# modelscope/FunASR

Measured on AMD Instinct MI355X. Metric: audio-seconds/sec (RTF^-1) Paraformer-large 30s@bs64, higher is better.
Workload: dtype f32 (GEMM / self-attention operands split into 2 fp16 planes, 3 fp16 MFMA products, f32 accumulate; all else f32)

## Files before the change

funasr_amd/_lib.py:

```python
from __future__ import annotations

import ctypes as C
import os
import subprocess
import threading

_HERE = os.path.dirname(os.path.abspath(__file__))
LIB_PATH = os.environ.get("PF_LIB_PATH") or os.path.join(_HERE, "libparaformer_hip.so")
CSRC_DIR = os.path.join(_HERE, "csrc")

ABI_VERSION = 5

_lock = threading.Lock()
_lib = None


class HipRuntimeError(RuntimeError):
    """A pf_* entry point returned a non-zero status."""


class pf_frontend_config(C.Structure):
    _fields_ = [
        ("sample_rate", C.c_int32), ("frame_length", C.c_int32), ("frame_shift", C.c_int32),
        ("n_mels", C.c_int32), ("lfr_m", C.c_int32), ("lfr_n", C.c_int32),
# ... 112 lines not shown
    "pf_predictor_destroy": (None, [_vp]),
    "pf_predictor_set_tensor": (C.c_int, [_vp, C.c_char_p, _vp, _i64]),
    "pf_predictor_missing": (C.c_int, [_vp]),
    "pf_predictor_alphas": (C.c_int, [_vp, _vp, _pi32, _i32, _i32, _vp, _vp, _pi32, _vp]),
    "pf_predictor_embeds": (C.c_int, [_vp, _vp, _i32, _i32, _i32, _vp, _vp]),
    "pf_predictor_alphas_begin": (C.c_int, [_vp, _i32, _vp, _pi32, _i32, _i32, _vp, _vp, _vp, _vp]),
    "pf_predictor_embeds_slot": (C.c_int, [_vp, _i32, _vp, _i32, _i32, _i32, _vp, _vp]),
    "pf_predictor_create_v3": (_vp, [C.POINTER(pf_predictor_config), C.POINTER(pf_predictor_v3_config)]),
    "pf_predictor_timestamp": (C.c_int, [_vp, _vp, _pi32, _pi32, _i32, _i32, _vp, _vp, _vp]),
    "pf_decoder_create": (_vp, [C.POINTER(pf_decoder_config)]),
    "pf_decoder_destroy": (None, [_vp]),
    "pf_decoder_set_decoders2": (C.c_int, [_vp, _i32]),
    "pf_decoder_set_tensor": (C.c_int, [_vp, C.c_char_p, _vp, _i64]),
    "pf_decoder_missing": (C.c_int, [_vp]),
    "pf_decoder_set_precision": (C.c_int, [_vp, _i32]),
    "pf_decoder_forward": (C.c_int, [_vp, _vp, _pi32, _vp, _pi32, _i32, _i32, _i32, _vp, _vp, _vp, _vp]),
    "pf_decoder_create_contextual": (_vp, [C.POINTER(pf_decoder_config)]),
    "pf_decoder_forward_contextual": (C.c_int, [_vp, _vp, _pi32, _vp, _pi32, _vp, _i32, _f32, _i32, _i32, _i32, _vp, _vp, _vp, _vp]),
    "pf_decoder_asf_scores": (C.c_int, [_vp, _vp, _pi32, _vp, _pi32, _i32, _i32, _i32, _i32, _vp, _vp]),
    "pf_vad_create": (_vp, [C.POINTER(pf_vad_config)]),
    "pf_vad_destroy": (None, [_vp]),
    "pf_vad_set_tensor": (C.c_int, [_vp, C.c_char_p, _vp, _i64]),
    "pf_vad_missing": (C.c_int, [_vp]),
    "pf_vad_forward": (C.c_int, [_vp, _vp, _i32, _i32, _vp, _pi32, _i32, _vp, _vp, _i32, _vp]),
    "pf_vad_frame_decibel": (C.c_int, [_vp, _i64, _i32, _i32, _i32, _vp, _vp]),
    "pf_vad_decision_create": (_vp, [C.POINTER(pf_vad_options)]),
    "pf_vad_decision_destroy": (None, [_vp]),
    "pf_vad_decision_set_thresholds": (None, [_vp, C.c_double, C.c_double]),
    "pf_vad_decision_state": (C.c_int, [_vp]),
    "pf_vad_decision_push": (C.c_int, [_vp, _vp, _vp, _i32, _i32, _i32, _vp, _i32]),
# ... 160 lines not shown
```

funasr_amd/csrc/attention_f16x2.hip:

```cpp
#include "common.h"

namespace pf {

namespace {

constexpr int DK = 128, KT = 32;
constexpr int KP_B = KT * DK * 2;
constexpr int VP_B = DK * KT * 2;
constexpr int STAGE_B = 2 * KP_B + 2 * VP_B;
constexpr int OLD = DK + 4;
constexpr int SLAB_B = 8 * 32 * OLD * 4;
constexpr int LDS_BYTES = SLAB_B > 3 * STAGE_B ? SLAB_B : 3 * STAGE_B;
constexpr float P_SCALE = 1024.f;
typedef _Float16 f16x8 __attribute__((ext_vector_type(8)));

constexpr float LAZY_TAU = 3.0f;
template <int PIPE, bool LAZY = false>
__global__ __launch_bounds__(512, 2) void attention_f16x2_kernel(Attn2Args p) {
    extern __shared__ __attribute__((aligned(16))) unsigned char smem[];
    constexpr int NSTAGE = PIPE ? 3 : 2;
    constexpr int QB = 256;
    constexpr int NV = 1;

    const int tid = threadIdx.x, lane = tid & 63;
    const int wave = __builtin_amdgcn_readfirstlane(tid >> 6);
    const int hh = lane >> 5, idx = lane & 31;
    int b, head, qblk;
    if (p.xcd_nqb > 0) {
        const int L = blockIdx.x, j = L >> 3;
        const int pair = (j / p.xcd_nqb) * 8 + (L & 7);
        if (pair >= p.B * p.H) return;
        qblk = j % p.xcd_nqb; head = pair % p.H; b = pair / p.H;
    } else {
        b = blockIdx.z; head = blockIdx.y; qblk = blockIdx.x;
    }
    const int Tq = p.qoffs ? p.qoffs[b + 1] - p.qoffs[b] : (p.Tq > 0 ? p.Tq : p.Tp);
    if (qblk * QB >= Tq) return;
// ... 44 lines not shown
            glds16(vsrc[v] + kt * KT, base + 2 * KP_B);
            glds16(vsrc[v] + p.vt_plane + kt * KT, base + 2 * KP_B + VP_B);
        }
    };

    const float sscale = p.sscale_dev ? p.sscale * *p.sscale_dev : p.sscale;
    const float sscale2 = LAZY ? sscale * 1.4426950408889634f : sscale;
#define PF_EXP(x_) (LAZY ? __builtin_amdgcn_exp2f(x_) : __expf(x_))
    constexpr float PSC = LAZY ? 1.f : P_SCALE;
    const int ntiles = (kend + KT - 1) / KT;

#define PF_QK(KT_, SA, SB)                                                                                            \
    {                                                                                                                 \
        const unsigned char* kp = smem + ((KT_) % NSTAGE) * STAGE_B + idx * 256;                                      \
        _Pragma("unroll") for (int r = 0; r < 16; ++r) { SA[r] = 0.f; SB[r] = 0.f; }                                  \
        _Pragma("unroll") for (int st = 0; st < 8; ++st) {                                                            \
            const int co = ((2 * st + hh) ^ (idx & 15)) * 16;                                                         \
            const f16x8 kh = __builtin_bit_cast(f16x8, *reinterpret_cast<const uint4*>(kp + co));                     \
            const f16x8 kl = __builtin_bit_cast(f16x8, *reinterpret_cast<const uint4*>(kp + KP_B + co));              \
            SA = __builtin_amdgcn_mfma_f32_32x32x16_f16(kl, qf[0][st], SA, 0, 0, 0);                                  \
            SB = __builtin_amdgcn_mfma_f32_32x32x16_f16(kh, qf[0][st], SB, 0, 0, 0);                                  \
            SA = __builtin_amdgcn_mfma_f32_32x32x16_f16(kh, qf[1][st], SA, 0, 0, 0);                                  \
        }                                                                                                             \
    }
#define PF_SOFTMAX(K0_, SA, SB)                                                                                       \
    {                                                                                                                 \
        float mx = -INFINITY;                                                                                         \
        if (LAZY && (K0_) >= kskip && (K0_) + KT <= kend) {         \
            _Pragma("unroll") for (int r = 0; r < 16; ++r) {                                                          \
                s[r] = (SA[r] + SB[r]) * sscale2;                                                                     \
                mx = fmaxf(mx, s[r]);                                                                                 \
            }                                                                                                         \
        } else {                                                                                                      \
            _Pragma("unroll") for (int r = 0; r < 16; ++r) {                                                          \
                const int key = (K0_) + (r & 3) + 8 * (r >> 2) + 4 * hh;                                              \
                s[r] = (unsigned)(key - kskip) < (unsigned)klen ? (SA[r] + SB[r]) * sscale2 : -INFINITY;              \
                mx = fmaxf(mx, s[r]);                                                                                 \
            }                                                                                                         \
        }                                                                                                             \
        mx = fmaxf(mx, __shfl_xor(mx, 32, 64));                                                                       \
        float m_new = fmaxf(m_run, mx);                                                                               \
// ... 5 lines not shown
        const float alpha = moved ? PF_EXP(m_run - m_new) : 1.f;                                                      \
        float psum = 0.f;                                                                                             \
        const float m_off = LAZY ? m_new - 10.f : m_new;          \
        _Pragma("unroll") for (int r = 0; r < 16; ++r) {                                                              \
            s[r] = PF_EXP(s[r] - m_off);                                                                              \
            psum += s[r];                                                                                             \
        }                                                                                                             \
        psum += __shfl_xor(psum, 32, 64);                                                                             \
        l_run = l_run * alpha + psum;                                                                                 \
        m_run = m_new;                                                                                                \
        if (!LAZY || __any(moved)) {                                                                                  \
            _Pragma("unroll") for (int d = 0; d < 4; ++d) _Pragma("unroll") for (int r = 0; r < 16; ++r) o[d][r] *= alpha; \
        }                                                                                                             \
    }
#define PF_PV(KT_)                                                                                                    \
    {                                                                                                                 \
        const unsigned char* vp = smem + ((KT_) % NSTAGE) * STAGE_B + 2 * KP_B + idx * 64;                            \
        _Pragma("unroll") for (int st = 0; st < 2; ++st) {                                                            \
            uint4 ph, pl;                                                                                             \
            split2_pk(s[8 * st + 0] * PSC, s[8 * st + 1] * PSC, ph.x, pl.x);                                  \
            split2_pk(s[8 * st + 2] * PSC, s[8 * st + 3] * PSC, ph.y, pl.y);                                  \
            split2_pk(s[8 * st + 4] * PSC, s[8 * st + 5] * PSC, ph.z, pl.z);                                  \
            split2_pk(s[8 * st + 6] * PSC, s[8 * st + 7] * PSC, ph.w, pl.w);                                  \
            const f16x8 Ph = __builtin_bit_cast(f16x8, ph), Pl = __builtin_bit_cast(f16x8, pl);                       \
            const int co = ((2 * st + hh) ^ ((idx >> 2) & 3)) * 16;                                                   \
            f16x8 vf[4][2];                                                                                           \
            _Pragma("unroll") for (int d = 0; d < 4; ++d) _Pragma("unroll") for (int pn = 0; pn < 2; ++pn)            \
                vf[d][pn] = __builtin_bit_cast(f16x8, *reinterpret_cast<const uint4*>(vp + pn * VP_B + d * 32 * 64 + co)); \
            _Pragma("unroll") for (int d = 0; d < 4; ++d) o[d] = __builtin_amdgcn_mfma_f32_32x32x16_f16(vf[d][1], Ph, o[d], 0, 0, 0); \
            _Pragma("unroll") for (int d = 0; d < 4; ++d) o[d] = __builtin_amdgcn_mfma_f32_32x32x16_f16(vf[d][0], Pl, o[d], 0, 0, 0); \
            _Pragma("unroll") for (int d = 0; d < 4; ++d) o[d] = __builtin_amdgcn_mfma_f32_32x32x16_f16(vf[d][0], Ph, o[d], 0, 0, 0); \
        }                                                                                                             \
    }

    float s[16];
    const bool active = qblk * QB + wave * 32 < Tq;
    if constexpr (PIPE == 0) {
        stage(0);
        for (int kt = 0; kt < ntiles; ++kt) {
            glds_wait_all();
            __syncthreads();
            if (kt + 1 < ntiles) stage(kt + 1);
            if (active) {
                floatx16 sa, sb;
                PF_QK(kt, sa, sb)
                PF_SOFTMAX(kt * KT, sa, sb)
                PF_PV(kt)
            }
        }
    } else {
        floatx16 ca, cb, na, nb;
        stage(0);
        if (ntiles > 1) stage(1);
        glds_wait_all();
        __syncthreads();
        PF_QK(0, ca, cb)
        for (int kt = 0; kt < ntiles; ++kt) {
            if (kt > 0) { glds_wait_all(); __syncthreads(); }
            if (kt + 2 < ntiles) stage(kt + 2);
            const int kn = kt + 1 < ntiles ? kt + 1 : kt;
            PF_QK(kn, na, nb)
            PF_SOFTMAX(kt * KT, ca, cb)
#pragma unroll
            for (int g = 0; g < 24; ++g) {
                __builtin_amdgcn_sched_group_barrier(0x008, 1, 0);
                __builtin_amdgcn_sched_group_barrier(0x002, 7, 0);
            }
            PF_PV(kt)
            ca = na; cb = nb;
        }
    }
#undef PF_QK
#undef PF_EXP
#undef PF_SOFTMAX
#undef PF_PV

    __syncthreads();
    float* slab = reinterpret_cast<float*>(smem) + wave * (32 * OLD);
    {
        const float inv = (LAZY ? p.oscale * P_SCALE : p.oscale) / l_run;
#pragma unroll
        for (int d = 0; d < 4; ++d)
#pragma unroll
            for (int g = 0; g < 4; ++g) {
                const float4 t = make_float4(o[d][4 * g + 0] * inv, o[d][4 * g + 1] * inv, o[d][4 * g + 2] * inv, o[d][4 * g + 3] * inv);
                *reinterpret_cast<float4*>(slab + idx * OLD + d * 32 + 8 * g + 4 * hh) = t;
            }
    }
    const int qw0 = qblk * QB + wave * 32;
#pragma unroll
    for (int it = 0; it < 8; ++it) {
        const int rr = it * 4 + (lane >> 4), c8 = (lane & 15) * 8;
// ... 2 lines not shown
        if (qw0 + rr < Tq) {
            uint4 h, l;
            split2_pk(a.x, a.y, h.x, l.x);
            split2_pk(a.z, a.w, h.y, l.y);
            split2_pk(c.x, c.y, h.z, l.z);
            split2_pk(c.z, c.w, h.w, l.w);
            unsigned short* op = p.O + (qrow0 + qw0 + rr) * p.ldo + head * DK + c8;
            *reinterpret_cast<uint4*>(op) = h;
            *reinterpret_cast<uint4*>(op + p.o_plane) = l;
        }
    }
}

}

int launch_attention_f16x2(const Attn2Args& a, hipStream_t stream) {
    PF_REQUIRE(a.B > 0 && a.H > 0 && (a.koffs || (a.Tp > 0 && a.Tp % 16 == 0)), "attention_f16x2: rows per sequence must be a positive multiple of 16");
    PF_REQUIRE(a.ldq % 8 == 0 && a.ldk % 8 == 0 && a.ldvt % 8 == 0 && a.ldo % 8 == 0 && a.q_plane % 8 == 0 &&
               a.k_plane % 8 == 0 && a.vt_plane % 8 == 0 && a.o_plane % 8 == 0, "attention_f16x2: strides % 8");
    PF_REQUIRE(((uintptr_t)a.Q & 15) == 0 && ((uintptr_t)a.K & 15) == 0 && ((uintptr_t)a.VT & 15) == 0 && ((uintptr_t)a.O & 15) == 0,
               "attention_f16x2: 16-B alignment");
    static PerDeviceOnce configured;
    if (!configured.done()) {
#if defined(PF_MEASUREMENT_KERNELS)
        PF_HIP_TRY(hipFuncSetAttribute(reinterpret_cast<const void*>(&attention_f16x2_kernel<0>),
                                       hipFuncAttributeMaxDynamicSharedMemorySize, LDS_BYTES));
        PF_HIP_TRY(hipFuncSetAttribute(reinterpret_cast<const void*>(&attention_f16x2_kernel<1>),
                                       hipFuncAttributeMaxDynamicSharedMemorySize, LDS_BYTES));
#endif
        PF_HIP_TRY(hipFuncSetAttribute(reinterpret_cast<const void*>(&attention_f16x2_kernel<0, true>),
                                       hipFuncAttributeMaxDynamicSharedMemorySize, LDS_BYTES));
        configured.mark();
    }
    const int rows = a.Tq > 0 ? a.Tq : a.Tp;
    Attn2Args k = a;
#if defined(PF_MEASUREMENT_KERNELS)
    PF_REQUIRE(a.variant == 0 || a.variant == 1 || a.variant == 3, "attention_f16x2: variant must be 0, 1 or 3");
#else
    PF_REQUIRE(a.variant == 3, "attention_f16x2: variant must be 3 (variants 0 / 1: the measurement library, make measure)");
#endif
    const int nqb = ceil_div(rows, 256);
    dim3 grid(nqb, a.H, a.B);
    k.xcd_nqb = (a.xcd_nqb >= 0 && nqb > 1) ? nqb : 0;
    if (k.xcd_nqb > 0) grid = dim3((unsigned)(ceil_div(a.B * a.H, 8) * 8 * nqb), 1, 1);
    if (a.variant == 3)
        hipLaunchKernelGGL((attention_f16x2_kernel<0, true>), grid, dim3(512), LDS_BYTES, stream, k);
#if defined(PF_MEASUREMENT_KERNELS)
    else if (a.variant == 1)
        hipLaunchKernelGGL(attention_f16x2_kernel<1>, grid, dim3(512), LDS_BYTES, stream, k);
    else
        hipLaunchKernelGGL(attention_f16x2_kernel<0>, grid, dim3(512), LDS_BYTES, stream, k);
#endif
    PF_HIP_TRY(hipGetLastError());
    return 0;
}

}
```

funasr_amd/csrc/common.h:

```cpp
#pragma once
#include <hip/hip_runtime.h>
#include <stdint.h>
#include <stdio.h>
#include <string>
#include <atomic>

typedef float floatx16 __attribute__((ext_vector_type(16)));
typedef float floatx4 __attribute__((ext_vector_type(4)));

namespace pf {

inline int current_device_slot() {
    int d = 0;
    if (hipGetDevice(&d) != hipSuccess || d < 0) d = 0;
    return d & 63;
}
struct PerDeviceOnce {
    std::atomic<bool> flag[64];
    PerDeviceOnce() { for (auto& f : flag) f.store(false, std::memory_order_relaxed); }
    bool done() const { return flag[current_device_slot()].load(std::memory_order_acquire); }
    void mark() { flag[current_device_slot()].store(true, std::memory_order_release); }
};
inline int device_cu_count() {
    static std::atomic<int> n[64];
// ... 344 lines not shown
struct Attn2Args {
    const unsigned short* Q; int ldq; size_t q_plane;
    const unsigned short* K; int ldk; size_t k_plane;
    const unsigned short* VT; int ldvt; size_t vt_plane;
    unsigned short* O; int ldo; size_t o_plane;
    const int* klens;
    int B, H, Tp;
    int Tq;
    float sscale;
    const float* sscale_dev;
    float oscale;
    int variant;
    const int* qoffs;
    int xcd_nqb;
    const int* koffs;
};
int launch_attention_f16x2(const Attn2Args& a, hipStream_t stream);

int launch_asf_scores(const float* Q, int ldq, const float* K, int ldk, float* P_scratch, float* out, int H, int dk, int N, int T,
                      int klen, float scale, hipStream_t stream);
bool attention_small_applicable(const AttnArgs& a, int dk);
int launch_attention_small(const AttnArgs& a, int dk, hipStream_t stream);
int launch_scatter_i32(const int* in, const int* map, int* out, int n, hipStream_t stream);
int launch_gather_rows(const float* table, int ld, int rows, const int* ids, float* out, int n, int D, hipStream_t stream);

int launch_vad_fsmn(const float* x, int ldx, const float* w, const float* cache_in, float* cache_out, float* y, int ldy,
                    int B, int T, int C, int L, int S, hipStream_t stream);
int launch_vad_softmax_sil(const float* x, int ldx, int M, int N, const int* ids, int n_ids, float* p_sil, float* probs,
                           int ldp, hipStream_t stream);
int launch_frame_decibel(const float* wav, int n_frames, int flen, int shift, float* out, hipStream_t stream);
// ... 3 lines not shown
```

funasr_amd/csrc/engine_decoder.hip:

```cpp
#include "engine_internal.h"

namespace pf {

std::string dec_layer_prefix(bool contextual, int n_blocks, int i) {
    return (contextual && i == n_blocks - 1) ? std::string("last_decoder.") : "decoders." + std::to_string(i) + ".";
}


int decoder_resolve(Decoder* d) {
    std::string first;
    const int miss = d->tt.missing(&first);
    if (miss) { set_error("decoder: " + std::to_string(miss) + " tensors not set, e.g. " + first); return -3; }
    d->layers.clear();
    for (int i = 0; i < d->cfg.n_blocks; ++i) {
        const std::string p = dec_layer_prefix(d->contextual, d->cfg.n_blocks, i);
        DecLayerW w;
        w.n1g = d->tt.get(p + "norm1.weight"); w.n1b = d->tt.get(p + "norm1.bias");
        w.w1 = d->tt.get(p + "feed_forward.w_1.weight"); w.b1 = d->tt.get(p + "feed_forward.w_1.bias");
        w.fng = d->tt.get(p + "feed_forward.norm.weight"); w.fnb = d->tt.get(p + "feed_forward.norm.bias");
        w.w2 = d->tt.get(p + "feed_forward.w_2.weight");
        w.n2g = d->tt.get(p + "norm2.weight"); w.n2b = d->tt.get(p + "norm2.bias");
        w.fsmn_w = d->tt.get(p + "self_attn.fsmn_block.weight");
        w.n3g = d->tt.get(p + "norm3.weight"); w.n3b = d->tt.get(p + "norm3.bias");
        w.q_w = d->tt.get(p + "src_attn.linear_q.weight"); w.q_b = d->tt.get(p + "src_attn.linear_q.bias");
// ... 627 lines not shown
    return 0;
}
int pf_decoder_set_tensor(pf_decoder* dh, const char* name, const float* data, int64_t numel) {
    Decoder* d = reinterpret_cast<Decoder*>(dh);
    PF_REQUIRE(d && name && data, "decoder_set_tensor: null");
    d->resolved = false;
    d->tt.drop_bf16();
    return d->tt.set(name, data, numel);
}
int pf_decoder_set_precision(pf_decoder* dh, int32_t mode) {
    Decoder* d = reinterpret_cast<Decoder*>(dh);
    PF_REQUIRE(d && mode >= 0 && mode <= 3, "decoder_set_precision: mode must be 0 (fp32 MFMA), 1 (bf16 operands), 2 (fp32 via bf16x3) or 3 (fp32 via f16x2)");
    d->precision = mode;
    return 0;
}
int pf_decoder_missing(const pf_decoder* dh) {
    const Decoder* d = reinterpret_cast<const Decoder*>(dh);
    return d ? d->tt.missing() : -1;
}

static int decoder_forward_impl(Decoder* d, const float* memory, const int32_t* mem_lens, const float* embeds,
                                const int32_t* tok_lens, int32_t B, int32_t T, int32_t N, float* logits, int32_t* ids,
                                float* hidden_out, hipStream_t s, int asf_layer, float* asf_scores, const DecCtxArgs* cx = nullptr);

int pf_decoder_forward(pf_decoder* dh, const float* memory, const int32_t* mem_lens, const float* embeds,
                       const int32_t* tok_lens, int32_t B, int32_t T, int32_t N, float* logits, int32_t* ids,
                       float* hidden_out, void* stream) {
    return decoder_forward_impl(reinterpret_cast<Decoder*>(dh), memory, mem_lens, embeds, tok_lens, B, T, N, logits, ids,
                                hidden_out, reinterpret_cast<hipStream_t>(stream), -1, nullptr);
}
// ... 152 lines not shown
                Gemm2Args g{};
                g.A = mem2; g.lda = D; g.a_plane = (size_t)Mkp * D; g.W = w.kv_2; g.ldw = D; g.w_plane = (size_t)2 * D * D;
                g.oscale = pow2f(-w.ew_kv); g.oscale_dev = dsc + 2; g.bias = w.kv_b; g.M = Mkp; g.N = 2 * D; g.K = D;
                g.qkv_D = D; g.kv_form = 1; g.Kp = k2; g.qk_plane = ((size_t)Mkp + 32) * D; g.VT = vt2; g.ldvt = Mkp + 64;
                g.vt_plane = (size_t)D * (Mkp + 64); g.k_mul = 1.f; g.v_mul = 1.f; g.kv_mul_dev = lsc;
                ProfScope ps(PROF_GEMM3, 2.0 * mem_rows * 2.0 * D * D, s);
                if ((rc = launch_gemm_f16x2(g, s))) return rc;
            }
            {
                Attn2Args aa{};
                aa.Q = d->q16.as<unsigned short>(); aa.ldq = D; aa.q_plane = (size_t)Mq * D;
                aa.K = k2; aa.ldk = D; aa.k_plane = ((size_t)Mkp + 32) * D; aa.VT = vt2; aa.ldvt = Mkp + 64;
                aa.vt_plane = (size_t)D * (Mkp + 64); aa.O = d->ctx16.as<unsigned short>(); aa.ldo = D; aa.o_plane = (size_t)Mq * D;
                aa.klens = d->mem_lens.as<int>(); aa.B = B; aa.H = c.n_heads; aa.Tp = Tp; aa.Tq = N; aa.qoffs = offs_dev;
                aa.sscale = pow2f(-w.e_q); aa.sscale_dev = lsc + 2; aa.oscale = pow2f(-10);
                aa.variant = 3;
                ProfScope ps(PROF_ATTN, 4.0 * tok_mem * D, s);
                if ((rc = launch_attention_f16x2(aa, s))) return rc;
            }
            if ((rc = gemm2_simple(d->ctx16.as<unsigned short>(), D, Mq, 0, w.o_2, w.ew_o, w.o_b, x, D, D, D, 0, x, D, s, lsc + 3)))
                return rc;
            continue;
        } else if (x3) {
            if ((rc = gemm3_simple(mem3, D, Mk, w3(lp + "src_attn.linear_k_v.weight", 2 * D, D), w.kv_b, d->kv.as<float>(),
                                   2 * D, 2 * D, D, 0, s))) return rc;
        } else if ((rc = gemm_simple(memory, D, w.kv_w, D, w.kv_b, d->kv.as<float>(), 2 * D, Mk, 2 * D, D, 0, nullptr, 0,
                                     nullptr, 0, s))) return rc;
        const bool ctx_block = cx && l == c.n_blocks - 1;
        if (ctx_block) {
            if (d->xself.ensure(sizeof(float) * (size_t)Mq * D) || d->xcat.ensure(sizeof(float) * (size_t)Mq * 2 * D)) return -2;
            PF_HIP_TRY(hipMemcpyAsync(d->xself.p, x, sizeof(float) * (size_t)Mq * D, hipMemcpyDeviceToDevice, s));
// ... 165 lines not shown
```

funasr_amd/csrc/engine_encoder.hip:

```cpp
#include "engine_internal.h"

namespace pf {

static void enc_layer_names(std::vector<std::pair<std::string, int>>& out, const pf_encoder_config& c) {
    out.push_back({"encoders0.0.", c.input_dim});
    for (int i = 0; i < c.n_blocks - 1; ++i) out.push_back({"encoders." + std::to_string(i) + ".", c.d_model});
    for (int i = 0; i < c.tp_blocks; ++i) out.push_back({"tp_encoders." + std::to_string(i) + ".", c.d_model});
}

int encoder_resolve(Encoder* e) {
    std::string first;
    const int miss = e->tt.missing(&first);
    if (miss) { set_error("encoder: " + std::to_string(miss) + " tensors not set, e.g. " + first); return -3; }
    std::vector<std::pair<std::string, int>> names;
    enc_layer_names(names, e->cfg);
    e->layers.clear();
    for (auto& nm : names) {
        const std::string& p = nm.first;
        EncLayerW w;
        w.prefix = p;
        w.in_dim = nm.second; w.in_pad = round_up(nm.second, 64);
        w.n1g = e->tt.get(p + "norm1.weight"); w.n1b = e->tt.get(p + "norm1.bias");
        w.qkv_w = e->tt.get(p + "self_attn.linear_q_k_v.weight"); w.qkv_b = e->tt.get(p + "self_attn.linear_q_k_v.bias");
        w.fsmn_w = e->tt.get(p + "self_attn.fsmn_block.weight");
// ... 443 lines not shown
int pf_encoder_set_option(pf_encoder* eh, const char* key, int32_t value) {
    Encoder* e = reinterpret_cast<Encoder*>(eh);
    PF_REQUIRE(e && key, "encoder_set_option: null");
    const std::string k = key;
    if (k == "fuse_row") { PF_REQUIRE(value == 0 || value == 1, "encoder_set_option: fuse_row is 0 or 1"); e->fuse_row = value; return 0; }
    if (k == "fsmn_fused") { PF_REQUIRE(value == 0 || value == 1, "encoder_set_option: fsmn_fused is 0 or 1"); e->fsmn_fused = value; return 0; }
    if (k == "w2_row") { PF_REQUIRE(value >= 0 && value <= 2, "encoder_set_option: w2_row is 0, 1 or 2"); e->w2_row = value; return 0; }
#if defined(PF_MEASUREMENT_KERNELS)
    if (k == "gemm_tile") { PF_REQUIRE(value == 0 || value == 1 || value == 2 || value == 5 || value == 6 || value == 7 || value == 8 || value == 9 || value == 10 || value == 12, "encoder_set_option: gemm_tile is 0, 1, 2, 5, 6, 7, 8, 9, 10 or 12"); e->gemm_tile = value; return 0; }
    if (k == "ffn_abl") { e->ffn_abl = value; return 0; }
    if (k == "ffn_fused") { PF_REQUIRE(value >= 0 && value <= 2, "encoder_set_option: ffn_fused is 0, 1 or 2"); e->ffn_fused = value; return 0; }
    if (k == "row_bm") { PF_REQUIRE(value == 0 || value == 96 || value == 128 || value == 129 || value == 130, "encoder_set_option: row_bm is 0, 96, 128, 129 or 130"); e->row_bm = value; return 0; }
    if (k == "row_sched") { PF_REQUIRE(value == 0 || value == 2, "encoder_set_option: row_sched is 0 or 2"); e->row_sched = value; return 0; }
    if (k == "w2_tile") { PF_REQUIRE(value == 0 || value == 2 || value == 7 || value == 8 || value == 10, "encoder_set_option: w2_tile is 0, 2, 7, 8 or 10"); e->w2_tile = value; return 0; }
    if (k == "row_nt") { PF_REQUIRE(value >= 0 && value <= 2, "encoder_set_option: row_nt is 0, 1 or 2"); e->row_nt = value; return 0; }
    if (k == "attn_variant") { PF_REQUIRE(value == 0 || value == 1 || value == 3, "encoder_set_option: attn_variant is 0, 1 or 3"); e->attn_variant = value; return 0; }
#else
    if (k == "gemm_tile") { PF_REQUIRE(value == 0 || value == 2 || value == 7 || value == 10, "encoder_set_option: gemm_tile is 0, 2, 7 or 10"); e->gemm_tile = value; return 0; }
    if (k == "ffn_abl" || k == "ffn_fused" || k == "row_bm" || k == "row_sched" || k == "w2_tile" || k == "row_nt" || k == "attn_variant") {
        set_error("encoder_set_option: " + k + " selects a measured-and-off shape: build and load the measurement library (make -C funasr_amd/csrc measure; PF_LIB_PATH)");
        return -1;
    }
#endif
    set_error("encoder_set_option: unknown key " + k);
    return -1;
}
static int poison(std::initializer_list<DevBuf*> bufs, int byte) {
    PF_HIP_TRY(hipDeviceSynchronize());
    for (DevBuf* b : bufs) if (b->p && b->cap) PF_HIP_TRY(hipMemset(b->p, byte, b->cap));
    PF_HIP_TRY(hipDeviceSynchronize());
    return 0;
}
int pf_encoder_debug_poison(pf_encoder* eh, int32_t byte) {
// ... 201 lines not shown
```

funasr_amd/csrc/engine_internal.h:

```cpp
#pragma once
#include <math.h>
#include <string.h>

#include <map>
#include <memory>
#include <mutex>
#include <string>
#include <vector>

#include "../../include/paraformer_hip.h"
#include "cif.h"
#include "lstm.h"
#include "common.h"
#include "frontend.h"
#include "stream.h"
#include "engine_tables.h"


namespace pf {

void set_error(const std::string& msg);
const char* get_error();

struct ProfRec { hipEvent_t a, b; int kind; double work; const char* tag; };
// ... 277 lines not shown
    bool vad_mask = false;
    std::vector<int32_t> h_vad;
    DevBuf vad_dev;
    int cur_mask_mode = 0;
    int fuse_row = 1;
    int fsmn_fused = 1;
    int ffn_fused = 0;
    int ffn_abl = 0;
    int row_bm = 0;
    int row_sched = 0;
    int w2_row = 2;
    int w2_tile = 7;
    DevBuf fs_grp;
    std::vector<int32_t> h_fs;
    const int* cur_fs = nullptr; int cur_fs_groups = 0;
    int attn_variant = 3;
    int row_nt = 1;
    double prof_rows = 0, prof_sq = 0;
    int gemm_tile = 0;
};


static inline int exp_for_bound(float bound) {
    if (!(bound > 0.f)) return 15;
    int e = (int)floorf(log2f(32768.f / bound));
    return e > 15 ? 15 : e;
}
static inline float pow2f(int e) { return ldexpf(1.f, e); }

static inline bool encoder_w2_row_form(const Encoder* e, int M) {
    if (e->w2_row != 2) return e->w2_row == 1;
// ... 50 lines not shown
};


struct Decoder {
    pf_decoder_config cfg;
    bool contextual = false;
    DevBuf xself, xcat, ctx_lens;
    TensorTable tt;
    std::vector<DecLayerW> layers;
    int n_blocks2 = 0;
    std::vector<DecLayerW> layers2;
    DecLayerW last;
    bool resolved = false;
    DevBuf x, t1, t2, ffn, ffn2, q, kv, ctx, mem_lens, tok_lens, pval, pidx, hid;
    int precision = 0;
    DevBuf t16, ffn16, ffn2_16, q16, kv16, ctx16, mem16, hid16;
    DevBuf dsc;
    DevBuf dscl, dlb;
    DevBuf k2, vt2;
    DevBuf splitk;
    bool lb_uploaded = false;
    int e_an = INT32_MIN;
    DevBuf asf_p;
    DevBuf offs_dev, map_dev, ids_packed;
    std::vector<int32_t> h_offs, h_map;
};


struct Ctc {
    int d_model, vocab;
// ... 117 lines not shown
```

funasr_amd/csrc/engine_kernels.hip:

```cpp
#include "engine_internal.h"

using namespace pf;

extern "C" {

int pf_k_gemm_skinny_ln(const float* A, int32_t lda, const float* W, int32_t ldw, const float* bias, const float* R2, int32_t ldr2,
                        float* Cout, int32_t ldc, int32_t M, int32_t N, int32_t K, int32_t relu, float* stats_out,
                        const float* stats_in, const float* ln_g, const float* ln_c, float ln_eps, const float* out_gamma, float* ws_part,
                        int32_t* ws_count, void* stream) {
    GemmArgs g{};
    g.ws_part = ws_part; g.ws_count = ws_count; g.ln_c1 = ln_c; g.ln_c2 = ln_c ? ln_c + N : nullptr; g.out_gamma = out_gamma;
    g.A = A; g.lda = lda; g.W = W; g.ldw = ldw; g.bias = bias; g.R2 = R2; g.ldr2 = ldr2; g.C = Cout; g.ldc = ldc;
    g.M = M; g.N = N; g.K = K; g.relu = relu; g.ln_stats_out = stats_out; g.ln_stats_in = stats_in; g.ln_g = ln_g; g.ln_eps = ln_eps;
    PF_REQUIRE(gemm_skinny_applicable(g), "gemm_skinny_ln: K % 16");
    return launch_gemm_skinny(g, reinterpret_cast<hipStream_t>(stream));
}
int pf_k_ln_consts(const float* W, int32_t ldw, int32_t N, int32_t K, const float* gamma, const float* beta, const float* bias, float* c,
                   void* stream) {
    return launch_ln_consts(W, ldw, N, K, gamma, beta, bias, c, c + N, reinterpret_cast<hipStream_t>(stream));
}
int pf_set_skinny_max_m(int32_t m) { g_skinny_max_m = m; return 0; }

int pf_k_gemm_f32(const float* A, int32_t lda, const float* W, int32_t ldw, const float* bias, const float* R1,
                  int32_t ldr1, const float* R2, int32_t ldr2, float* C, int32_t ldc, int32_t M, int32_t N, int32_t K,
// ... 121 lines not shown
    return 0;
}
int pf_k_attention_f16x2(const void* Q2, int64_t q_plane, const void* K2, int64_t k_plane, const void* VT2, int32_t ldvt,
                         int64_t vt_plane, void* O2, int64_t o_plane, const int32_t* klens_dev, int32_t B, int32_t H,
                         int32_t Tp, int32_t Tq, float sscale, float oscale, int32_t variant, int32_t iters, float* ms_out,
                         void* stream) {
    hipStream_t s = reinterpret_cast<hipStream_t>(stream);
    Attn2Args aa{};
    const int D = H * 128;
    aa.Q = reinterpret_cast<const unsigned short*>(Q2); aa.ldq = D; aa.q_plane = (size_t)q_plane;
    aa.K = reinterpret_cast<const unsigned short*>(K2); aa.ldk = D; aa.k_plane = (size_t)k_plane;
    aa.VT = reinterpret_cast<const unsigned short*>(VT2); aa.ldvt = ldvt; aa.vt_plane = (size_t)vt_plane;
    aa.O = reinterpret_cast<unsigned short*>(O2); aa.ldo = D; aa.o_plane = (size_t)o_plane;
    aa.klens = klens_dev; aa.B = B; aa.H = H; aa.Tp = Tp; aa.Tq = Tq; aa.sscale = sscale; aa.oscale = oscale;
    aa.variant = variant & 15; aa.xcd_nqb = (variant & 16) ? -1 : 0;
    int rc;
    if (iters <= 0 || !ms_out) return launch_attention_f16x2(aa, s);
    for (int i = 0; i < 3; ++i) if ((rc = launch_attention_f16x2(aa, s))) return rc;
    hipEvent_t a, b;
    PF_HIP_TRY(hipEventCreate(&a));
    PF_HIP_TRY(hipEventCreate(&b));
    PF_HIP_TRY(hipEventRecord(a, s));
    for (int i = 0; i < iters; ++i) if ((rc = launch_attention_f16x2(aa, s))) return rc;
    PF_HIP_TRY(hipEventRecord(b, s));
    PF_HIP_TRY(hipEventSynchronize(b));
    float ms = 0.f;
    PF_HIP_TRY(hipEventElapsedTime(&ms, a, b));
    (void)hipEventDestroy(a);
    (void)hipEventDestroy(b);
    *ms_out = ms / iters;
// ... 231 lines not shown
```

funasr_amd/paraformer_decoder.py:

```python
from __future__ import annotations

from typing import List

import torch
import torch.nn as nn

from . import _lib
from .hip_module import Holder, HipModule, ParamHolder, depthwise, device_lens, host_i32, layer_norm, linear, stream_ptr
from .register import tables


def _ffn(block, d_model, ffn):
    block.norm1 = layer_norm(d_model)
    block.feed_forward = Holder()
    block.feed_forward.w_1 = linear(ffn, d_model)
    block.feed_forward.norm = layer_norm(ffn)
    block.feed_forward.w_2 = linear(d_model, ffn, bias=False)


def _block2(d_model, ffn, kernel_size):
    b = Holder()
    _ffn(b, d_model, ffn)
    b.norm2 = layer_norm(d_model)
    b.self_attn = Holder()
# ... 49 lines not shown
        self.output_layer = linear(vocab_size, D) if use_output_layer else None

    def _default_precision(self) -> str:
        ok = self.d_model % 256 == 0 and self.d_model // self.attention_heads == 128 and self.linear_units % 256 == 0
        return "f16x2" if ok else "fp32"

    def _mode(self) -> str:
        return getattr(self, "_precision", None) or self._default_precision()

    def set_precision(self, mode=None):
        if mode is not None and mode not in ("fp32", "bf16", "bf16x3", "f16x2"):
            raise ValueError("precision must be 'fp32', 'bf16', 'bf16x3' or 'f16x2'")
        self._precision = mode
        return self

    def _make_config(self):
        return _lib.pf_decoder_config(self.vocab_size if self.output_layer is not None else 0, self.d_model, self.attention_heads, self.linear_units,
                                      self.att_layer_num, self.kernel_size, self.sanm_shfit, 1e-12)

    def _after_create(self, lib, handle):
        if self.decoders2 is not None:
            _lib.check(lib.pf_decoder_set_decoders2(handle, len(self.decoders2)), "pf_decoder_set_decoders2")

    def _apply_settings(self):
        lib, h = self._ensure_handle()
        _lib.check(lib.pf_decoder_set_precision(h, {"fp32": 0, "bf16": 1, "bf16x3": 2, "f16x2": 3}[self._mode()]),
                   "pf_decoder_set_precision")
        return lib, h

    def _run(self, hs_pad, hlens, ys_in_pad, ys_in_lens, want_logits: bool, want_ids: bool, want_hidden: bool = False):
        lib, h = self._apply_settings()
        dev = self._handle_device
        mem = hs_pad.to(device=dev, dtype=torch.float32).contiguous()
        emb = ys_in_pad.to(device=dev, dtype=torch.float32).contiguous()
        B, T, D = mem.shape
        N = emb.shape[1]
        mlen_c, _ = host_i32(hlens, B)
        tlen_c, tlens = host_i32(ys_in_lens, B)
        logits = torch.empty(B, N, self.vocab_size, device=dev, dtype=torch.float32) if want_logits else None
        ids = torch.empty(B, N, device=dev, dtype=torch.int32) if want_ids else None
        hid = torch.empty(B, N, D, device=dev, dtype=torch.float32) if want_hidden else None
        with torch.cuda.device(dev):
# ... 42 lines not shown
```

include/paraformer_hip.h:

```cpp
#ifndef PARAFORMER_HIP_H_
#define PARAFORMER_HIP_H_

#include <stdint.h>

#ifdef __cplusplus
extern "C" {
#endif

#define PF_ABI_VERSION 5

const char* pf_last_error(void);
int pf_abi_version(void);
int pf_device_count(void);

int pf_set_concurrency_guard(int32_t on);
int pf_concurrency_guard(void);

typedef struct pf_frontend pf_frontend;

typedef struct pf_frontend_config {
    int32_t sample_rate;
    int32_t frame_length;
    int32_t frame_shift;
    int32_t n_mels;
// ... 96 lines not shown
    int32_t d_model;
    int32_t n_heads;
    int32_t ffn_dim;
    int32_t n_blocks;
    int32_t kernel_size;
    int32_t sanm_shift;
    float ln_eps;
} pf_decoder_config;

pf_decoder* pf_decoder_create(const pf_decoder_config* cfg);
void pf_decoder_destroy(pf_decoder* d);
int pf_decoder_set_decoders2(pf_decoder* d, int32_t n_layers);
int pf_decoder_set_tensor(pf_decoder* d, const char* name, const float* data, int64_t numel);
int pf_decoder_missing(const pf_decoder* d);
int pf_decoder_set_precision(pf_decoder* d, int32_t mode);
int pf_decoder_forward(pf_decoder* d, const float* memory_dev, const int32_t* mem_lens_host,
                       const float* embeds_dev, const int32_t* tok_lens_host, int32_t B, int32_t T, int32_t N,
                       float* logits_dev, int32_t* ids_dev, float* hidden_dev, void* stream);
typedef struct pf_paraformer pf_paraformer;
pf_paraformer* pf_paraformer_create(pf_encoder* e, pf_predictor* p, pf_decoder* d);
void pf_paraformer_destroy(pf_paraformer* m);
int pf_paraformer_forward(pf_paraformer* m, const float* feats_dev, const int32_t* lens_host, int32_t B, int32_t T,
                          const float* pe_dev, int32_t* ids_dev, int32_t ids_ld, int32_t* token_num_host,
                          float* alphas_dev, float* peaks_dev, void* stream);
int pf_paraformer_begin(pf_paraformer* m, const float* feats_dev, const int32_t* lens_host, int32_t B, int32_t T,
                        const float* pe_dev, void* stream);
int pf_paraformer_finish(pf_paraformer* m, int32_t ticket, int32_t* ids_dev, int32_t ids_ld, int32_t* token_num_host,
                         float* alphas_dev, float* peaks_dev, void* stream);
const float* pf_paraformer_encoder_out(const pf_paraformer* m);
const float* pf_paraformer_embeds(const pf_paraformer* m);
// ... 251 lines not shown
```

Baseline: 39100.

## Add 4-wave attention variant with auto selection and batched K-fragment loads

Adds a 4-wave (128-query block) form of the f16x2 flash-attention kernel and a default variant 7 that picks it when the workgroup-round count across CUs favours smaller blocks, targeting tail and underfill waste at batch 64. The QK loop now loads four K fragment pairs before issuing their MFMAs, with sched_group_barrier hints, and the PV loop also gets these hints, to overlap LDS reads with matrix work. It also adds ablation and staggered-wave measurement variants, a decoder set_option entry point and host-side qlens for packed decoder rows. The heuristic uses a fixed 1.15 factor and the extra live fragments can raise register pressure.

```diff
diff --git a/funasr_amd/_lib.py b/funasr_amd/_lib.py
--- a/funasr_amd/_lib.py
+++ b/funasr_amd/_lib.py
@@ -150,6 +150,7 @@
     "pf_decoder_set_tensor": (C.c_int, [_vp, C.c_char_p, _vp, _i64]),
     "pf_decoder_missing": (C.c_int, [_vp]),
     "pf_decoder_set_precision": (C.c_int, [_vp, _i32]),
+    "pf_decoder_set_option": (C.c_int, [_vp, C.c_char_p, _i32]),
     "pf_decoder_forward": (C.c_int, [_vp, _vp, _pi32, _vp, _pi32, _i32, _i32, _i32, _vp, _vp, _vp, _vp]),
     "pf_decoder_create_contextual": (_vp, [C.POINTER(pf_decoder_config)]),
     "pf_decoder_forward_contextual": (C.c_int, [_vp, _vp, _pi32, _vp, _pi32, _vp, _i32, _f32, _i32, _i32, _i32, _vp, _vp, _vp, _vp]),
diff --git a/funasr_amd/csrc/attention_f16x2.hip b/funasr_amd/csrc/attention_f16x2.hip
--- a/funasr_amd/csrc/attention_f16x2.hip
+++ b/funasr_amd/csrc/attention_f16x2.hip
@@ -11,16 +11,19 @@
 constexpr int OLD = DK + 4;
 constexpr int SLAB_B = 8 * 32 * OLD * 4;
 constexpr int LDS_BYTES = SLAB_B > 3 * STAGE_B ? SLAB_B : 3 * STAGE_B;
+constexpr int SLAB4_B = 4 * 32 * OLD * 4;
+constexpr int LDS4_BYTES = SLAB4_B > 2 * STAGE_B ? SLAB4_B : 2 * STAGE_B;
 constexpr float P_SCALE = 1024.f;
 typedef _Float16 f16x8 __attribute__((ext_vector_type(8)));
 
 constexpr float LAZY_TAU = 3.0f;
-template <int PIPE, bool LAZY = false>
-__global__ __launch_bounds__(512, 2) void attention_f16x2_kernel(Attn2Args p) {
+template <int PIPE, bool LAZY = false, int NW = 8, int STAG = 0, int ABL = 0>
+__global__ __launch_bounds__(NW * 64, 2) void attention_f16x2_kernel(Attn2Args p) {
     extern __shared__ __attribute__((aligned(16))) unsigned char smem[];
-    constexpr int NSTAGE = PIPE ? 3 : 2;
-    constexpr int QB = 256;
-    constexpr int NV = 1;
+    static_assert((NW == 8 || NW == 4) && (STAG == 0 || (PIPE == 0 && NW == 8)), "attention_f16x2: form");
+    constexpr int NSTAGE = (PIPE || STAG == 1) ? 3 : 2;
+    constexpr int QB = NW * 32;
+    constexpr int NV = 8 / NW;
 
     const int tid = threadIdx.x, lane = tid & 63;
     const int wave = __builtin_amdgcn_readfirstlane(tid >> 6);
@@ -95,17 +98,37 @@
     {                                                                                                                 \
         const unsigned char* kp = smem + ((KT_) % NSTAGE) * STAGE_B + idx * 256;                                      \
         _Pragma("unroll") for (int r = 0; r < 16; ++r) { SA[r] = 0.f; SB[r] = 0.f; }                                  \
-        _Pragma("unroll") for (int st = 0; st < 8; ++st) {                                                            \
+        if constexpr (ABL & 4) { asm volatile("" : "+v"(SA), "+v"(SB)); }   \
+        else if constexpr (ABL & 64) { _Pragma("unroll") for (int st = 0; st < 8; ++st) {                             \
             const int co = ((2 * st + hh) ^ (idx & 15)) * 16;                                                         \
             const f16x8 kh = __builtin_bit_cast(f16x8, *reinterpret_cast<const uint4*>(kp + co));                     \
             const f16x8 kl = __builtin_bit_cast(f16x8, *reinterpret_cast<const uint4*>(kp + KP_B + co));              \
             SA = __builtin_amdgcn_mfma_f32_32x32x16_f16(kl, qf[0][st], SA, 0, 0, 0);                                  \
             SB = __builtin_amdgcn_mfma_f32_32x32x16_f16(kh, qf[0][st], SB, 0, 0, 0);                                  \
             SA = __builtin_amdgcn_mfma_f32_32x32x16_f16(kh, qf[1][st], SA, 0, 0, 0);                                  \
-        }                                                                                                             \
+        } }                                                                                                           \
+        else { _Pragma("unroll") for (int h4 = 0; h4 < 8; h4 += 4) {   \
+            f16x8 kh[4], kl[4];                                        \
+            _Pragma("unroll") for (int j = 0; j < 4; ++j) {                                                           \
+                const int co = ((2 * (h4 + j) + hh) ^ (idx & 15)) * 16;                                               \
+                kh[j] = __builtin_bit_cast(f16x8, *reinterpret_cast<const uint4*>(kp + co));                          \
+                kl[j] = __builtin_bit_cast(f16x8, *reinterpret_cast<const uint4*>(kp + KP_B + co));                   \
+            }                                                                                                         \
+            _Pragma("unroll") for (int j = 0; j < 4; ++j) {                                                           \
+                SA = __builtin_amdgcn_mfma_f32_32x32x16_f16(kl[j], qf[0][h4 + j], SA, 0, 0, 0);                       \
+                SB = __builtin_amdgcn_mfma_f32_32x32x16_f16(kh[j], qf[0][h4 + j], SB, 0, 0, 0);                       \
+                SA = __builtin_amdgcn_mfma_f32_32x32x16_f16(kh[j], qf[1][h4 + j], SA, 0, 0, 0);                       \
+            }                                                                                                         \
+             \
+            __builtin_amdgcn_sched_group_barrier(0x100, 8, 0);                                                        \
+            __builtin_amdgcn_sched_group_barrier(0x008, 12, 0);                                                       \
+        } }                                                                                                           \
     }
 #define PF_SOFTMAX(K0_, SA, SB)                                                                                       \
-    {                                                                                                                 \
+    if constexpr (ABL & 1) {                                                                                          \
+        _Pragma("unroll") for (int r = 0; r < 16; ++r) s[r] = (SA[r] + SB[r]) * sscale2;                              \
+        l_run += 1.f;                                                                                                 \
+    } else {                                                                                                          \
         float mx = -INFINITY;                                                                                         \
         if (LAZY && (K0_) >= kskip && (K0_) + KT <= kend) {         \
             _Pragma("unroll") for (int r = 0; r < 16; ++r) {                                                          \
@@ -141,7 +164,7 @@
         }                                                                                                             \
     }
 #define PF_PV(KT_)                                                                                                    \
-    {                                                                                                                 \
+    if constexpr (!(ABL & 2)) {                                                                                       \
         const unsigned char* vp = smem + ((KT_) % NSTAGE) * STAGE_B + 2 * KP_B + idx * 64;                            \
         _Pragma("unroll") for (int st = 0; st < 2; ++st) {                                                            \
             uint4 ph, pl;                                                                                             \
@@ -157,24 +180,35 @@
             _Pragma("unroll") for (int d = 0; d < 4; ++d) o[d] = __builtin_amdgcn_mfma_f32_32x32x16_f16(vf[d][1], Ph, o[d], 0, 0, 0); \
             _Pragma("unroll") for (int d = 0; d < 4; ++d) o[d] = __builtin_amdgcn_mfma_f32_32x32x16_f16(vf[d][0], Pl, o[d], 0, 0, 0); \
             _Pragma("unroll") for (int d = 0; d < 4; ++d) o[d] = __builtin_amdgcn_mfma_f32_32x32x16_f16(vf[d][0], Ph, o[d], 0, 0, 0); \
+            if constexpr (PIPE == 0 && !(ABL & 64)) {            \
+                __builtin_amdgcn_sched_group_barrier(0x100, 8, 0);                                                    \
+                __builtin_amdgcn_sched_group_barrier(0x008, 12, 0);                                                   \
+            }                                                                                                         \
         }                                                                                                             \
     }
 
     float s[16];
     const bool active = qblk * QB + wave * 32 < Tq;
     if constexpr (PIPE == 0) {
+        constexpr bool NO_DMA = (ABL & 8) != 0;
         stage(0);
+        if constexpr (NO_DMA) for (int t = 1; t < NSTAGE && t < ntiles; ++t) stage(t);
+        if constexpr (STAG == 2) { if (wave >= 4) __builtin_amdgcn_s_setprio(1); }
+        const bool late = STAG == 1 && wave >= 4;
+        if constexpr (!(ABL & 32)) __builtin_amdgcn_s_waitcnt(0x0F70);
         for (int kt = 0; kt < ntiles; ++kt) {
             glds_wait_all();
             __syncthreads();
-            if (kt + 1 < ntiles) stage(kt + 1);
+            if (!NO_DMA && kt + 1 < ntiles) stage(kt + 1);
             if (active) {
                 floatx16 sa, sb;
+                if (late && kt > 0) PF_PV(kt - 1)
                 PF_QK(kt, sa, sb)
                 PF_SOFTMAX(kt * KT, sa, sb)
-                PF_PV(kt)
+                if (!late) PF_PV(kt)
             }
         }
+        if (late && active && ntiles > 0) PF_PV(ntiles - 1)
     } else {
         floatx16 ca, cb, na, nb;
         stage(0);
@@ -203,6 +237,15 @@
 #undef PF_PV
 
     __syncthreads();
+    if constexpr (ABL & 16) {
+        float acc = l_run;
+#pragma unroll
+        for (int d = 0; d < 4; ++d)
+#pragma unroll
+            for (int r = 0; r < 16; ++r) acc += o[d][r];
+        if (acc == 12345.678f) p.O[(qrow0 + qc) * p.ldo + head * DK] = 1;
+        return;
+    }
     float* slab = reinterpret_cast<float*>(smem) + wave * (32 * OLD);
     {
         const float inv = (LAZY ? p.oscale * P_SCALE : p.oscale) / l_run;
@@ -235,42 +278,91 @@
 
 }
 
+static int attn2_workgroups(const Attn2Args& a, int rows, int qb) {
+    long n = 0;
+    for (int b = 0; b < a.B; ++b) n += ceil_div(a.qlens_host ? a.qlens_host[b] : rows, qb);
+    return (int)(n * a.H);
+}
+static bool attn2_takes_four_waves(const Attn2Args& a, int rows) {
+    const int n_cu = device_cu_count();
+    const int rounds8 = ceil_div(attn2_workgroups(a, rows, 256), n_cu), rounds4 = ceil_div(attn2_workgroups(a, rows, 128), 2 * n_cu);
+    return 1.15 * rounds4 < 1.0 * rounds8;
+}
+
 int launch_attention_f16x2(const Attn2Args& a, hipStream_t stream) {
     PF_REQUIRE(a.B > 0 && a.H > 0 && (a.koffs || (a.Tp > 0 && a.Tp % 16 == 0)), "attention_f16x2: rows per sequence must be a positive multiple of 16");
     PF_REQUIRE(a.ldq % 8 == 0 && a.ldk % 8 == 0 && a.ldvt % 8 == 0 && a.ldo % 8 == 0 && a.q_plane % 8 == 0 &&
                a.k_plane % 8 == 0 && a.vt_plane % 8 == 0 && a.o_plane % 8 == 0, "attention_f16x2: strides % 8");
     PF_REQUIRE(((uintptr_t)a.Q & 15) == 0 && ((uintptr_t)a.K & 15) == 0 && ((uintptr_t)a.VT & 15) == 0 && ((uintptr_t)a.O & 15) == 0,
                "attention_f16x2: 16-B alignment");
+#define PF_ATTN2_LDS(KERNEL, BYTES) \
+    PF_HIP_TRY(hipFuncSetAttribute(reinterpret_cast<const void*>(&KERNEL), hipFuncAttributeMaxDynamicSharedMemorySize, BYTES))
     static PerDeviceOnce configured;
     if (!configured.done()) {
 #if defined(PF_MEASUREMENT_KERNELS)
-        PF_HIP_TRY(hipFuncSetAttribute(reinterpret_cast<const void*>(&attention_f16x2_kernel<0>),
-                                       hipFuncAttributeMaxDynamicSharedMemorySize, LDS_BYTES));
-        PF_HIP_TRY(hipFuncSetAttribute(reinterpret_cast<const void*>(&attention_f16x2_kernel<1>),
-                                       hipFuncAttributeMaxDynamicSharedMemorySize, LDS_BYTES));
+        PF_ATTN2_LDS(attention_f16x2_kernel<0>, LDS_BYTES);
+        PF_ATTN2_LDS(attention_f16x2_kernel<1>, LDS_BYTES);
+        PF_ATTN2_LDS((attention_f16x2_kernel<0, true, 8, 2>), LDS_BYTES);
+        PF_ATTN2_LDS((attention_f16x2_kernel<0, true, 8, 0, 1>), LDS_BYTES);
+        PF_ATTN2_LDS((attention_f16x2_kernel<0, true, 8, 0, 2>), LDS_BYTES);
+        PF_ATTN2_LDS((attention_f16x2_kernel<0, true, 8, 0, 4>), LDS_BYTES);
+        PF_ATTN2_LDS((attention_f16x2_kernel<0, true, 8, 0, 8>), LDS_BYTES);
+        PF_ATTN2_LDS((attention_f16x2_kernel<0, true, 8, 0, 16>), LDS_BYTES);
+        PF_ATTN2_LDS((attention_f16x2_kernel<0, true, 8, 0, 32>), LDS_BYTES);
+        PF_ATTN2_LDS((attention_f16x2_kernel<0, true, 8, 0, 64>), LDS_BYTES);
+        PF_ATTN2_LDS((attention_f16x2_kernel<0, true, 8, 1>), LDS_BYTES);
 #endif
-        PF_HIP_TRY(hipFuncSetAttribute(reinterpret_cast<const void*>(&attention_f16x2_kernel<0, true>),
-                                       hipFuncAttributeMaxDynamicSharedMemorySize, LDS_BYTES));
+        PF_ATTN2_LDS((attention_f16x2_kernel<0, true>), LDS_BYTES);
+        PF_ATTN2_LDS((attention_f16x2_kernel<0, true, 4>), LDS4_BYTES);
         configured.mark();
     }
+#undef PF_ATTN2_LDS
     const int rows = a.Tq > 0 ? a.Tq : a.Tp;
+    if (a.qlens_host)
+        for (int b = 0; b < a.B; ++b) PF_REQUIRE(a.qlens_host[b] >= 0 && a.qlens_host[b] <= rows, "attention_f16x2: qlens_host out of range");
     Attn2Args k = a;
 #if defined(PF_MEASUREMENT_KERNELS)
-    PF_REQUIRE(a.variant == 0 || a.variant == 1 || a.variant == 3, "attention_f16x2: variant must be 0, 1 or 3");
+    PF_REQUIRE(a.variant == 0 || a.variant == 1 || (a.variant >= 3 && a.variant <= 7), "attention_f16x2: variant must be 0, 1 or 3 .. 7");
+    PF_REQUIRE(a.abl == 0 || (a.variant == 3 && (a.abl == 1 || a.abl == 2 || a.abl == 4 || a.abl == 8 || a.abl == 16 || a.abl == 32 || a.abl == 64)),
+               "attention_f16x2: abl is 1, 2, 4, 8, 16, 32 or 64, on variant 3");
 #else
-    PF_REQUIRE(a.variant == 3, "attention_f16x2: variant must be 3 (variants 0 / 1: the measurement library, make measure)");
+    PF_REQUIRE(a.variant == 3 || a.variant == 5 || a.variant == 7,
+               "attention_f16x2: variant must be 3, 5 or 7 (variants 0 / 1 / 4 / 6: the measurement library, make measure)");
+    PF_REQUIRE(a.abl == 0, "attention_f16x2: ablation builds are in the measurement library (make measure)");
 #endif
-    const int nqb = ceil_div(rows, 256);
+    const int variant = a.variant != 7 ? a.variant : attn2_takes_four_waves(a, rows) ? 5 : 3;
+    const int qb = variant == 5 ? 128 : 256, threads = variant == 5 ? 256 : 512;
+    const int nqb = ceil_div(rows, qb);
     dim3 grid(nqb, a.H, a.B);
     k.xcd_nqb = (a.xcd_nqb >= 0 && nqb > 1) ? nqb : 0;
     if (k.xcd_nqb > 0) grid = dim3((unsigned)(ceil_div(a.B * a.H, 8) * 8 * nqb), 1, 1);
-    if (a.variant == 3)
-        hipLaunchKernelGGL((attention_f16x2_kernel<0, true>), grid, dim3(512), LDS_BYTES, stream, k);
+    if (variant == 5)
+        hipLaunchKernelGGL((attention_f16x2_kernel<0, true, 4>), grid, dim3(threads), LDS4_BYTES, stream, k);
+    else if (variant == 3 && a.abl == 0)
+        hipLaunchKernelGGL((attention_f16x2_kernel<0, true>), grid, dim3(threads), LDS_BYTES, stream, k);
 #if defined(PF_MEASUREMENT_KERNELS)
-    else if (a.variant == 1)
-        hipLaunchKernelGGL(attention_f16x2_kernel<1>, grid, dim3(512), LDS_BYTES, stream, k);
+    else if (variant == 3 && a.abl == 1)
+        hipLaunchKernelGGL((attention_f16x2_kernel<0, true, 8, 0, 1>), grid, dim3(threads), LDS_BYTES, stream, k);
+    else if (variant == 3 && a.abl == 2)
+        hipLaunchKernelGGL((attention_f16x2_kernel<0, true, 8, 0, 2>), grid, dim3(threads), LDS_BYTES, stream, k);
+    else if (variant == 3 && a.abl == 4)
+        hipLaunchKernelGGL((attention_f16x2_kernel<0, true, 8, 0, 4>), grid, dim3(threads), LDS_BYTES, stream, k);
+    else if (variant == 3 && a.abl == 8)
+        hipLaunchKernelGGL((attention_f16x2_kernel<0, true, 8, 0, 8>), grid, dim3(threads), LDS_BYTES, stream, k);
+    else if (variant == 3 && a.abl == 16)
+        hipLaunchKernelGGL((attention_f16x2_kernel<0, true, 8, 0, 16>), grid, dim3(threads), LDS_BYTES, stream, k);
+    else if (variant == 3 && a.abl == 32)
+        hipLaunchKernelGGL((attention_f16x2_kernel<0, true, 8, 0, 32>), grid, dim3(threads), LDS_BYTES, stream, k);
+    else if (variant == 3)
+        hipLaunchKernelGGL((attention_f16x2_kernel<0, true, 8, 0, 64>), grid, dim3(threads), LDS_BYTES, stream, k);
+    else if (variant == 4)
+        hipLaunchKernelGGL((attention_f16x2_kernel<0, true, 8, 1>), grid, dim3(threads), LDS_BYTES, stream, k);
+    else if (variant == 6)
+        hipLaunchKernelGGL((attention_f16x2_kernel<0, true, 8, 2>), grid, dim3(threads), LDS_BYTES, stream, k);
+    else if (variant == 1)
+        hipLaunchKernelGGL(attention_f16x2_kernel<1>, grid, dim3(threads), LDS_BYTES, stream, k);
     else
-        hipLaunchKernelGGL(attention_f16x2_kernel<0>, grid, dim3(512), LDS_BYTES, stream, k);
+        hipLaunchKernelGGL(attention_f16x2_kernel<0>, grid, dim3(threads), LDS_BYTES, stream, k);
 #endif
     PF_HIP_TRY(hipGetLastError());
     return 0;
diff --git a/funasr_amd/csrc/common.h b/funasr_amd/csrc/common.h
--- a/funasr_amd/csrc/common.h
+++ b/funasr_amd/csrc/common.h
@@ -382,6 +382,8 @@
     const int* qoffs;
     int xcd_nqb;
     const int* koffs;
+    const int* qlens_host;
+    int abl;
 };
 int launch_attention_f16x2(const Attn2Args& a, hipStream_t stream);
 
diff --git a/funasr_amd/csrc/engine_decoder.hip b/funasr_amd/csrc/engine_decoder.hip
--- a/funasr_amd/csrc/engine_decoder.hip
+++ b/funasr_amd/csrc/engine_decoder.hip
@@ -665,6 +665,22 @@
     d->precision = mode;
     return 0;
 }
+int pf_decoder_set_option(pf_decoder* dh, const char* key, int32_t value) {
+    Decoder* d = reinterpret_cast<Decoder*>(dh);
+    PF_REQUIRE(d && key, "decoder_set_option: null");
+    const std::string k(key);
+    if (k == "attn_variant") {
+#if defined(PF_MEASUREMENT_KERNELS)
+        PF_REQUIRE(value >= 3 && value <= 7, "decoder_set_option: attn_variant is 3 .. 7");
+#else
+        PF_REQUIRE(value == 3 || value == 5 || value == 7, "decoder_set_option: attn_variant is 3, 5 or 7 (4 / 6: the measurement library)");
+#endif
+        d->attn_variant = value;
+        return 0;
+    }
+    set_error("decoder_set_option: unknown key " + k);
+    return -1;
+}
 int pf_decoder_missing(const pf_decoder* dh) {
     const Decoder* d = reinterpret_cast<const Decoder*>(dh);
     return d ? d->tt.missing() : -1;
@@ -847,7 +863,7 @@
                 aa.vt_plane = (size_t)D * (Mkp + 64); aa.O = d->ctx16.as<unsigned short>(); aa.ldo = D; aa.o_plane = (size_t)Mq * D;
                 aa.klens = d->mem_lens.as<int>(); aa.B = B; aa.H = c.n_heads; aa.Tp = Tp; aa.Tq = N; aa.qoffs = offs_dev;
                 aa.sscale = pow2f(-w.e_q); aa.sscale_dev = lsc + 2; aa.oscale = pow2f(-10);
-                aa.variant = 3;
+                aa.variant = d->attn_variant; aa.qlens_host = pack ? tok_lens : nullptr;
                 ProfScope ps(PROF_ATTN, 4.0 * tok_mem * D, s);
                 if ((rc = launch_attention_f16x2(aa, s))) return rc;
             }
diff --git a/funasr_amd/csrc/engine_encoder.hip b/funasr_amd/csrc/engine_encoder.hip
--- a/funasr_amd/csrc/engine_encoder.hip
+++ b/funasr_amd/csrc/engine_encoder.hip
@@ -481,9 +481,10 @@
     if (k == "row_sched") { PF_REQUIRE(value == 0 || value == 2, "encoder_set_option: row_sched is 0 or 2"); e->row_sched = value; return 0; }
     if (k == "w2_tile") { PF_REQUIRE(value == 0 || value == 2 || value == 7 || value == 8 || value == 10, "encoder_set_option: w2_tile is 0, 2, 7, 8 or 10"); e->w2_tile = value; return 0; }
     if (k == "row_nt") { PF_REQUIRE(value >= 0 && value <= 2, "encoder_set_option: row_nt is 0, 1 or 2"); e->row_nt = value; return 0; }
-    if (k == "attn_variant") { PF_REQUIRE(value == 0 || value == 1 || value == 3, "encoder_set_option: attn_variant is 0, 1 or 3"); e->attn_variant = value; return 0; }
+    if (k == "attn_variant") { PF_REQUIRE(value == 0 || value == 1 || (value >= 3 && value <= 7), "encoder_set_option: attn_variant is 0, 1 or 3 .. 7"); e->attn_variant = value; return 0; }
 #else
     if (k == "gemm_tile") { PF_REQUIRE(value == 0 || value == 2 || value == 7 || value == 10, "encoder_set_option: gemm_tile is 0, 2, 7 or 10"); e->gemm_tile = value; return 0; }
+    if (k == "attn_variant" && (value == 3 || value == 5 || value == 7)) { e->attn_variant = value; return 0; }
     if (k == "ffn_abl" || k == "ffn_fused" || k == "row_bm" || k == "row_sched" || k == "w2_tile" || k == "row_nt" || k == "attn_variant") {
         set_error("encoder_set_option: " + k + " selects a measured-and-off shape: build and load the measurement library (make -C funasr_amd/csrc measure; PF_LIB_PATH)");
         return -1;
diff --git a/funasr_amd/csrc/engine_internal.h b/funasr_amd/csrc/engine_internal.h
--- a/funasr_amd/csrc/engine_internal.h
+++ b/funasr_amd/csrc/engine_internal.h
@@ -315,7 +315,7 @@
     DevBuf fs_grp;
     std::vector<int32_t> h_fs;
     const int* cur_fs = nullptr; int cur_fs_groups = 0;
-    int attn_variant = 3;
+    int attn_variant = 7;
     int row_nt = 1;
     double prof_rows = 0, prof_sq = 0;
     int gemm_tile = 0;
@@ -396,6 +396,7 @@
     bool resolved = false;
     DevBuf x, t1, t2, ffn, ffn2, q, kv, ctx, mem_lens, tok_lens, pval, pidx, hid;
     int precision = 0;
+    int attn_variant = 7;
     DevBuf t16, ffn16, ffn2_16, q16, kv16, ctx16, mem16, hid16;
     DevBuf dsc;
     DevBuf dscl, dlb;
diff --git a/funasr_amd/csrc/engine_kernels.hip b/funasr_amd/csrc/engine_kernels.hip
--- a/funasr_amd/csrc/engine_kernels.hip
+++ b/funasr_amd/csrc/engine_kernels.hip
@@ -159,6 +159,7 @@
     aa.O = reinterpret_cast<unsigned short*>(O2); aa.ldo = D; aa.o_plane = (size_t)o_plane;
     aa.klens = klens_dev; aa.B = B; aa.H = H; aa.Tp = Tp; aa.Tq = Tq; aa.sscale = sscale; aa.oscale = oscale;
     aa.variant = variant & 15; aa.xcd_nqb = (variant & 16) ? -1 : 0;
+    aa.abl = (variant >> 8) & 127;
     int rc;
     if (iters <= 0 || !ms_out) return launch_attention_f16x2(aa, s);
     for (int i = 0; i < 3; ++i) if ((rc = launch_attention_f16x2(aa, s))) return rc;
diff --git a/funasr_amd/paraformer_decoder.py b/funasr_amd/paraformer_decoder.py
--- a/funasr_amd/paraformer_decoder.py
+++ b/funasr_amd/paraformer_decoder.py
@@ -87,6 +87,12 @@
         self._precision = mode
         return self
 
+    def set_option(self, key: str, value: int):
+        if not hasattr(self, "_options"):
+            self._options = {}
+        self._options[str(key)] = int(value)
+        return self
+
     def _make_config(self):
         return _lib.pf_decoder_config(self.vocab_size if self.output_layer is not None else 0, self.d_model, self.attention_heads, self.linear_units,
                                       self.att_layer_num, self.kernel_size, self.sanm_shfit, 1e-12)
@@ -99,6 +105,8 @@
         lib, h = self._ensure_handle()
         _lib.check(lib.pf_decoder_set_precision(h, {"fp32": 0, "bf16": 1, "bf16x3": 2, "f16x2": 3}[self._mode()]),
                    "pf_decoder_set_precision")
+        for key, value in getattr(self, "_options", {}).items():
+            _lib.check(lib.pf_decoder_set_option(h, key.encode(), int(value)), "pf_decoder_set_option")
         return lib, h
 
     def _run(self, hs_pad, hlens, ys_in_pad, ys_in_lens, want_logits: bool, want_ids: bool, want_hidden: bool = False):
diff --git a/include/paraformer_hip.h b/include/paraformer_hip.h
--- a/include/paraformer_hip.h
+++ b/include/paraformer_hip.h
@@ -134,6 +134,7 @@
 int pf_decoder_set_tensor(pf_decoder* d, const char* name, const float* data, int64_t numel);
 int pf_decoder_missing(const pf_decoder* d);
 int pf_decoder_set_precision(pf_decoder* d, int32_t mode);
+int pf_decoder_set_option(pf_decoder* d, const char* key, int32_t value);
 int pf_decoder_forward(pf_decoder* d, const float* memory_dev, const int32_t* mem_lens_host,
                        const float* embeds_dev, const int32_t* tok_lens_host, int32_t B, int32_t T, int32_t N,
                        float* logits_dev, int32_t* ids_dev, float* hidden_dev, void* stream);
```

New measurement: 39100 (median of 4 runs). No clear change (+0.0%).
